# BerserkerMother/Video-Summarization

Hardware: AMD Instinct MI355X
Metric: frames/sec scored (whole node), synthetic [B,T=1024,D=1024] (higher is better)
Workload: dtype f32; 1 GPU; configs[2]: B=64 videos x T=1024 frames x D=1024 per GPU, scorer cfg M-A (heads 4, d_model 256, layers 4), logits + hidden state; global_batch=64, parallelism=videos sharded over 1 GPU(s), no all_gather of scores

## Files before the change

### video-summarization_amd/csrc/vs_kernels.hip

```cpp
#include "vs_train_device.h"
#include "vs_kernels.h"
#include "vs_launch.h"

namespace {

enum { EPI_BIAS = 0, EPI_RELU = 1, EPI_PE = 2, EPI_QKV = 3,
       EPI_GATE = 4,
       EPI_RELU_DROP = 5 };
struct EpiArgs {
    unsigned long long seed;
    unsigned site;
    float p;
    float scale;
};

__device__ __forceinline__ unsigned long long stamp() { return vs_stamp(); }

template <int EPI, int NWM = 2, int DIAG = 0, int NJ = 2, int PREC = 0, int C16 = 0, int KW = 32, int A16 = 0>
__global__ __launch_bounds__(128 * NWM, 2) void gemm_nt_128(
    const float *__restrict__ A, const float *__restrict__ W, const float *__restrict__ bias,
    float *__restrict__ C, int M, int N, int K, const float *__restrict__ pe, int T, int H, int dh,
    unsigned long long *__restrict__ diag = nullptr, EpiArgs ea = EpiArgs{0ull, 0u, 0.f, 0.f}) {
    static_assert(KW == 32 || (KW == 64 && (PREC == 1 || PREC == 3)), "64-wide k-tiles exist for the 16-bit operands only");
    static_assert(A16 == 0 || PREC == 1 || PREC == 3, "16-bit-stored A belongs to the 16-bit operand modes");
// ... 476 lines not shown
            const float v = (PREC == 2 ? acc[j][t] * (1.0f / F16X3_WS) : acc[j][t]) + bj[j] + res[(size_t)row * N + cbase + 32 * j];
            acc[j][t] = v;
            s += v;
        }
        part[t] = half_sum(s);
    }
    if (r == 0) {
#pragma unroll
        for (int t = 0; t < 16; ++t) red[wc * 64 + 32 * wr + acc_row(t, h)] = part[t];
    }
    __syncthreads();
    float mean[16];
#pragma unroll
    for (int t = 0; t < 16; ++t) {
        const int rl = 32 * wr + acc_row(t, h);
        mean[t] = (red[rl] + red[64 + rl]) * (1.0f / N);
    }
    __syncthreads();
#pragma unroll
    for (int t = 0; t < 16; ++t) {
        float s = 0.f;
#pragma unroll
        for (int j = 0; j < NB; ++j) { const float c = acc[j][t] - mean[t]; acc[j][t] = c; s += c * c; }
        part[t] = half_sum(s);
    }
    if (r == 0) {
#pragma unroll
        for (int t = 0; t < 16; ++t) red[wc * 64 + 32 * wr + acc_row(t, h)] = part[t];
    }
    __syncthreads();
#pragma unroll
    for (int t = 0; t < 16; ++t) {
        const int rl = 32 * wr + acc_row(t, h);
        const float rstd = 1.0f / sqrtf((red[rl] + red[64 + rl]) * (1.0f / N) + 1e-5f);
        const int row = m0 + rl;
#pragma unroll
        for (int j = 0; j < NB; ++j) {
            const float y = acc[j][t] * rstd * gj[j] + bej[j];
            acc[j][t] = y;
            if (row < M) out[(size_t)row * N + cbase + 32 * j] = y;
        }
    }
    if (score_w != nullptr) {
        for (int c = 0; c < num_classes; ++c) {
            __syncthreads();
            float wj[NB];
#pragma unroll
            for (int j = 0; j < NB; ++j) wj[j] = score_w[(size_t)c * N + cbase + 32 * j];
#pragma unroll
            for (int t = 0; t < 16; ++t) {
                float s = 0.f;
#pragma unroll
                for (int j = 0; j < NB; ++j) s += acc[j][t] * wj[j];
                part[t] = half_sum(s);
            }
            if (r == 0) {
#pragma unroll
                for (int t = 0; t < 16; ++t) red[wc * 64 + 32 * wr + acc_row(t, h)] = part[t];
            }
            __syncthreads();
            if (tid < 64) {
                const int row = m0 + tid;
                if (row < M) {
                    float s = red[tid] + red[64 + tid] + score_b[c];
                    if (sigmoid) s = 1.0f / (1.0f + expf(-s));
                    scores[(size_t)row * num_classes + c] = s;
                }
            }
        }
    }
}

struct LnTail {
    const float *W2, *b2;
    float *C2;
    int T, H, dhs;
};
struct LnPhase2 {
    const float *W, *bias, *gamma, *beta;
    float *out;
    LnTail tl;
};

template <int NT, int PREC, int A16, int DIAG, int TAIL>
__device__ __forceinline__ void ln_rows_tiles(
    const float *__restrict__ A, const float *__restrict__ W, const float *__restrict__ bias,
    const float *__restrict__ res, const float *__restrict__ gamma, const float *__restrict__ beta,
    float *__restrict__ out, int M, int K,
    const float *__restrict__ score_w, const float *__restrict__ score_b, int num_classes,
    int sigmoid, float *__restrict__ scores, unsigned long long *__restrict__ diag, const LnTail tl, const LnPhase2 p2) {
    static_assert(TAIL == 0 || (NT == 8 && PREC == 0 && DIAG == 0), "the register-fed tail exists for exact fp32 at d_model 256");
    constexpr int BM = 128, N = 32 * NT, BK = 16, LD = BK + 4;
    constexpr int WL = (N * BK / 4 + 255) / 256;
    constexpr bool TWO = TAIL >= 3;
    constexpr int NPH = TWO ? 2 : 1;
    constexpr int TN2 = TAIL == 2 ? 3 * N : 4 * N;
    constexpr int SMALL2 = TAIL == 3 ? 3 * N + 3 * N : TAIL == 4 ? 3 * N : 0;
    __shared__ __attribute__((aligned(16))) float smem[2 * (BM + N) * LD + 4 * N + (TAIL != 0 ? TN2 : 0) + SMALL2];
    float *gam_s = smem + 2 * (BM + N) * LD, *bet_s = gam_s + N, *sw_s = bet_s + N, *bias_s = sw_s + N;
    float *bias2_s = bias_s + N;
    float *small2_s = bias2_s + TN2;

    int tid = threadIdx.x, lane = tid & 63, wave = tid >> 6;
    int r = lane & 31, h = lane >> 5;
    const int ntiles = (M + BM - 1) / BM;
    const int nk = K / BK;

    constexpr float SC = PREC == 2 ? F16X3_WS : 1.0f;
    for (int i = tid; i < N; i += 256) { gam_s[i] = gamma[i]; bet_s[i] = beta[i]; bias_s[i] = bias[i] * SC; }
    if constexpr (TAIL != 0)
        for (int i = tid; i < TN2; i += 256) bias2_s[i] = tl.b2[i];
    if constexpr (TWO) {
        for (int i = tid; i < N; i += 256) { small2_s[i] = p2.gamma[i]; small2_s[N + i] = p2.beta[i]; small2_s[2 * N + i] = p2.bias[i]; }
        if constexpr (TAIL == 3)
            for (int i = tid; i < 3 * N; i += 256) small2_s[3 * N + i] = p2.tl.b2[i];
    }

    int lrow = tid >> 2, lc4 = (tid & 3) * 4;
    f32x4 pa[2], pw[WL];
    u32x2 pa16[2];
    const float *aptr[2], *wptr[WL];
    const unsigned short *aptr16[2];
#pragma unroll
    for (int i = 0; i < WL; ++i) {
        int wrow = lrow + 64 * i; wrow = wrow < N ? wrow : N - 1;
        wptr[i] = W + (size_t)wrow * K + lc4;
    }
    static_assert(PREC != 0 || N % 64 == 0, "the exact-fp32 staging map covers W without a guard");
    __amdgpu_buffer_rsrc_t ars = __builtin_amdgcn_make_buffer_rsrc(const_cast<float *>(A), 0, 0, 0x00020000);
    __amdgpu_buffer_rsrc_t wrs = __builtin_amdgcn_make_buffer_rsrc(const_cast<float *>(W), 0, N * K * 4, 0x00020000);
    int aoff[2], woff[WL];
#pragma unroll
    for (int i = 0; i < WL; ++i) woff[i] = ((lrow + 64 * i) * K + lc4) * 4;
    auto gload = [&](int i, int kb) __attribute__((always_inline)) {
        if (i < 2) pa[i] = __builtin_bit_cast(f32x4, __builtin_amdgcn_raw_buffer_load_b128(ars, aoff[i], kb, 0));
        else pw[i - 2] = __builtin_bit_cast(f32x4, __builtin_amdgcn_raw_buffer_load_b128(wrs, woff[i - 2], kb, 0));
    };
    constexpr int LDB = 12;
    auto stage = [&](int buf) __attribute__((always_inline)) {
        float *As = smem + buf * (BM + N) * LD, *Ws = As + BM * LD;
        if constexpr (PREC == 2) {
#pragma unroll
            for (int i = 0; i < 2; ++i) {
                u32x2 hi, lo;
                split_f16x4((const float *)&pa[i], hi, lo);
                *(u32x2 *)&As[(lrow + 64 * i) * LD + lc4 / 2] = hi;
                *(u32x2 *)&As[(lrow + 64 * i) * LD + 8 + lc4 / 2] = lo;
            }
#pragma unroll
            for (int i = 0; i < WL; ++i)
                if (lrow + 64 * i < N) {
                    u32x2 hi, lo;
                    const f32x4 ws = pw[i] * F16X3_WS;
                    split_f16x4((const float *)&ws, hi, lo);
                    *(u32x2 *)&Ws[(lrow + 64 * i) * LD + lc4 / 2] = hi;
                    *(u32x2 *)&Ws[(lrow + 64 * i) * LD + 8 + lc4 / 2] = lo;
                }
        } else if constexpr (PREC == 1) {
#pragma unroll
            for (int i = 0; i < 2; ++i) {
                u32x2 u;
                if constexpr (A16 != 0) u = pa16[i];
                else { u[0] = pack_bf16(pa[i][0], pa[i][1]); u[1] = pack_bf16(pa[i][2], pa[i][3]); }
                *(u32x2 *)&As[(lrow + 64 * i) * LDB + lc4 / 2] = u;
            }
#pragma unroll
            for (int i = 0; i < WL; ++i)
                if (lrow + 64 * i < N) {
                    u32x2 u; u[0] = pack_bf16(pw[i][0], pw[i][1]); u[1] = pack_bf16(pw[i][2], pw[i][3]);
                    *(u32x2 *)&Ws[(lrow + 64 * i) * LDB + lc4 / 2] = u;
                }
        } else {
#pragma unroll
            for (int i = 0; i < 2; ++i) *(f32x4 *)&As[(lrow + 64 * i) * LD + lc4] = pa[i];
#pragma unroll
            for (int i = 0; i < WL; ++i) *(f32x4 *)&Ws[(lrow + 64 * i) * LD + lc4] = pw[i];
        }
    };

    f32x16 acc[NT];

    constexpr int TCH = 128, TWB = 4 * 32 * 36, TBUF = TCH * 36;
    static_assert(TAIL == 0 || TWB + 2 * TBUF <= 2 * (BM + N) * LD, "corners and weight tiles fit the staging area");
    int r2 = tid >> 3, c2 = (tid & 7) * 4;
    __amdgpu_buffer_rsrc_t wrs2 = __builtin_amdgcn_make_buffer_rsrc(const_cast<float *>(tl.W2), 0, TN2 * N * 4, 0x00020000);
    const float *tbias_s = bias2_s;
    int woff2 = (r2 * N + c2) * 4;
    f32x4 pw2[4];
    f32x16 U[4];
    auto tail_soff = [&](int c, int kt) __attribute__((always_inline)) { return (TCH * c * N + 32 * kt) * 4; };
    auto tail_load = [&](int i, int soff) __attribute__((always_inline)) {
        pw2[i] = __builtin_bit_cast(f32x4, __builtin_amdgcn_raw_buffer_load_b128(wrs2, woff2, soff + 32 * i * N * 4, 0));
    };
    auto tail_stage = [&](int buf) __attribute__((always_inline)) {
#pragma unroll
        for (int i = 0; i < 4; ++i) *(f32x4 *)&smem[TWB + buf * TBUF + (r2 + 32 * i) * 36 + c2] = pw2[i];
    };
    auto bias_mfma = [&](int c) __attribute__((always_inline)) {
        const f32x16 zero = {0.f, 0.f, 0.f, 0.f, 0.f, 0.f, 0.f, 0.f, 0.f, 0.f, 0.f, 0.f, 0.f, 0.f, 0.f, 0.f};
#pragma unroll
        for (int jj = 0; jj < 4; ++jj) {
            const float bv = tbias_s[TCH * c + 32 * jj + r];
            U[jj] = MFMA32(h == 0 ? bv : 0.f, 1.0f, zero);
        }
    };
    auto tail_step = [&](auto ktc, int nsoff) __attribute__((always_inline)) {
        constexpr int kt = decltype(ktc)::value;
        const float *wp = smem + TWB + (kt & 1) * TBUF + r * 36 + 4 * h;
        float *wd = smem + TWB + ((kt + 1) & 1) * TBUF + r2 * 36 + c2;
        f32x4 fw[3];
        fw[0] = *(const f32x4 *)wp;
        fw[1] = *(const f32x4 *)(wp + 32 * 36);
        __builtin_amdgcn_sched_barrier(0);
#pragma unroll
        for (int t = 0; t < 16; ++t) {
            const int g = t / 4, jj = t % 4;
            if (t + 2 < 16) fw[(t + 2) % 3] = *(const f32x4 *)(wp + 32 * ((t + 2) % 4) * 36 + 8 * ((t + 2) / 4));
            if (t < 4) tail_load(t, nsoff);
            if (t >= 12) *(f32x4 *)(wd + 32 * (t - 12) * 36) = pw2[t - 12];
#pragma unroll
            for (int s2 = 0; s2 < 4; ++s2) U[jj] = MFMA32(fw[t % 3][s2], acc[kt][4 * g + s2], U[jj]);
            __builtin_amdgcn_sched_group_barrier(0x008, 1, 0);
            if (t + 2 < 16) __builtin_amdgcn_sched_group_barrier(0x100, 1, 0);
            if (t < 4) __builtin_amdgcn_sched_group_barrier(0x020, 1, 0);
            __builtin_amdgcn_sched_group_barrier(0x008, 3, 0);
            if (t >= 12) __builtin_amdgcn_sched_group_barrier(0x200, 1, 0);
            __builtin_amdgcn_sched_barrier(0);
        }
        __syncthreads();
    };

    unsigned long long dsum[3] = {0, 0, 0}, tbegin = 0, tq = 0, ktiles = 0;
    if constexpr (DIAG != 0) tbegin = stamp();
    for (int tile = blockIdx.x; tile < ntiles; tile += gridDim.x) {
        if constexpr (DIAG != 0) tq = stamp();
        const int m0 = tile * BM;
      static_for<NPH>([&](auto phc) __attribute__((always_inline)) {
        constexpr int PH = decltype(phc)::value;
        constexpr bool P1 = TWO && PH == 1;
        constexpr int PT = !TWO ? TAIL : PH == 0 ? 1 : TAIL == 3 ? 2 : 0;
        constexpr int PTN2 = PT == 2 ? 3 * N : 4 * N, TNC = PTN2 / TCH;
        const LnTail ptl = P1 ? p2.tl : tl;
        const float *pA = P1 ? tl.C2 : A;
        const int pK = P1 ? 4 * N : K, pnk = P1 ? 4 * N / BK : nk;
        const float *pgam_s = P1 ? small2_s : gam_s, *pbet_s = P1 ? small2_s + N : bet_s, *pbias_s = P1 ? small2_s + 2 * N : bias_s;
        float *pout = P1 ? p2.out : out;
        if constexpr (TWO) {
            asm volatile("" : "+v"(tid));
            lane = tid & 63; wave = tid >> 6; r = lane & 31; h = lane >> 5;
            lrow = tid >> 2; lc4 = (tid & 3) * 4; r2 = tid >> 3; c2 = (tid & 7) * 4; woff2 = (r2 * N + c2) * 4;
            wrs = __builtin_amdgcn_make_buffer_rsrc(const_cast<float *>(P1 ? p2.W : W), 0, N * pK * 4, 0x00020000);
#pragma unroll
            for (int i = 0; i < WL; ++i) woff[i] = ((lrow + 64 * i) * pK + lc4) * 4;
            if constexpr (PT != 0) {
                wrs2 = __builtin_amdgcn_make_buffer_rsrc(const_cast<float *>(ptl.W2), 0, PTN2 * N * 4, 0x00020000);
                tbias_s = P1 ? small2_s + 3 * N : bias2_s;
            }
        }
        int row = m0 + 32 * wave + r;
        const bool row_ok = row < M;
        row = row_ok ? row : M - 1;
#pragma unroll
        for (int i = 0; i < 2; ++i) {
            int ar = m0 + lrow + 64 * i; ar = ar < M ? ar : M - 1;
            if constexpr (A16 != 0) {
                aptr16[i] = (const unsigned short *)A + (size_t)ar * K + lc4;
                pa16[i] = *(const u32x2 *)aptr16[i];
            } else if constexpr (PREC == 0) {
                aoff[i] = ((ar - m0) * pK + lc4) * 4;
            } else {
                aptr[i] = A + (size_t)ar * K + lc4;
                pa[i] = *(const f32x4 *)aptr[i];
            }
        }
        if constexpr (PREC == 0) {
            ars = __builtin_amdgcn_make_buffer_rsrc(const_cast<float *>(pA + (size_t)m0 * pK), 0, (M - m0 < BM ? M - m0 : BM) * pK * 4, 0x00020000);
            if constexpr (P1) {
#pragma unroll
                for (int i = 2; i < 2 + WL; ++i) gload(i, 0);
                asm volatile("s_waitcnt vmcnt(0)" ::: "memory");
                __builtin_amdgcn_fence(__ATOMIC_RELEASE, "workgroup");
                __syncthreads();
                __builtin_amdgcn_fence(__ATOMIC_ACQUIRE, "workgroup");
#pragma unroll
                for (int i = 0; i < 2; ++i) gload(i, 0);
            } else {
#pragma unroll
                for (int i = 0; i < 2 + WL; ++i) gload(i, 0);
            }
        } else {
#pragma unroll
            for (int i = 0; i < WL; ++i) pw[i] = *(const f32x4 *)wptr[i];
        }
        if constexpr (!P1) {
            const float *rp = res + (size_t)row * N + 4 * h;
#pragma unroll
            for (int j = 0; j < NT; ++j)
#pragma unroll
                for (int q = 0; q < 4; ++q) {
                    f32x4 rv = *(const f32x4 *)(rp + 32 * j + 8 * q);
                    if constexpr (PREC == 2) rv *= SC;
#pragma unroll
                    for (int e = 0; e < 4; ++e) acc[j][4 * q + e] = rv[e];
                }
        }
        if constexpr (!P1) __syncthreads();
        stage(0);
        __syncthreads();
        if constexpr (DIAG != 0) { dsum[2] += stamp() - tq; ktiles += nk; }

        for (int kt = 0; kt < pnk; ++kt) {
            const int kn = kt + 1 < pnk ? kt + 1 : kt;
            const float *As = smem + (kt & 1) * (BM + N) * LD, *Ws = As + BM * LD;
            if constexpr (PREC == 2) {
                const float *arow = As + (32 * wave + r) * LD + 4 * h;
                const f16x8 ah = __builtin_bit_cast(f16x8, *(const u32x4 *)arow);
                const f16x8 al = __builtin_bit_cast(f16x8, *(const u32x4 *)(arow + 8));
#pragma unroll
                for (int i = 0; i < 2; ++i) pa[i] = *(const f32x4 *)(aptr[i] + kn * BK);
#pragma unroll
                for (int i = 0; i < WL; ++i) pw[i] = *(const f32x4 *)(wptr[i] + kn * BK);
#pragma unroll
                for (int j = 0; j < NT; ++j) {
                    const float *wrow = Ws + (32 * j + r) * LD + 4 * h;
                    const f16x8 wh = __builtin_bit_cast(f16x8, *(const u32x4 *)wrow);
                    const f16x8 wl = __builtin_bit_cast(f16x8, *(const u32x4 *)(wrow + 8));
                    acc[j] = MFMA_F16(wl, ah, acc[j]);
                    acc[j] = MFMA_F16(wh, al, acc[j]);
                    acc[j] = MFMA_F16(wh, ah, acc[j]);
                }
                stage((kt + 1) & 1);
                __syncthreads();
                continue;
            }
            if constexpr (PREC == 1) {
                const bf16x8 fa = __builtin_bit_cast(bf16x8, *(const u32x4 *)(As + (32 * wave + r) * LDB + 4 * h));
#pragma unroll
                for (int i = 0; i < 2; ++i) {
                    if constexpr (A16 != 0) pa16[i] = *(const u32x2 *)(aptr16[i] + kn * BK);
                    else pa[i] = *(const f32x4 *)(aptr[i] + kn * BK);
                }
#pragma unroll
                for (int i = 0; i < WL; ++i) pw[i] = *(const f32x4 *)(wptr[i] + kn * BK);
#pragma unroll
                for (int j = 0; j < NT; ++j) {
                    const bf16x8 fw = __builtin_bit_cast(bf16x8, *(const u32x4 *)(Ws + (32 * j + r) * LDB + 4 * h));
                    acc[j] = MFMA_BF16(fw, fa, acc[j]);
                }
                stage((kt + 1) & 1);
                __syncthreads();
                continue;
            }
            const float *ap = As + (32 * wave + r) * LD + 4 * h;
            const float *wp = Ws + r * LD + 4 * h;
            constexpr int NS = 2 * NT, NL = 2 + WL;
            constexpr int LPS = (NL + NT - 1) / NT;
            constexpr int WB = NS - (NL + LPS - 1) / LPS;
            static_assert(BK == 16 && (NL + LPS - 1) / LPS <= NT, "loads and LDS writes of a k-tile occupy distinct steps");
            f32x4 fa[2], fw[3];
            fa[0] = *(const f32x4 *)ap;
            fw[0] = *(const f32x4 *)wp;
            fw[1] = *(const f32x4 *)(wp + 32 * LD);
            fa[1] = *(const f32x4 *)(ap + 8);
            __builtin_amdgcn_sched_barrier(0);
#pragma unroll
            for (int t = 0; t < NS; ++t) {
                const int g = t / NT, j = t % NT;
                if (t + 2 < NS) fw[(t + 2) % 3] = *(const f32x4 *)(wp + 32 * ((t + 2) % NT) * LD + 8 * ((t + 2) / NT));
                int nld = 0, nwr = 0;
#pragma unroll
                for (int q = 0; q < LPS; ++q) {
                    const int il = t * LPS + q, iw = (t - WB) * LPS + q;
                    if (il < NL) { gload(il, kn * (BK * 4)); ++nld; }
                    if (t >= WB && iw < NL) {
                        float *Ad = smem + ((kt + 1) & 1) * (BM + N) * LD, *Wd = Ad + BM * LD;
                        if (iw < 2) *(f32x4 *)&Ad[(lrow + 64 * iw) * LD + lc4] = pa[iw];
                        else *(f32x4 *)&Wd[(lrow + 64 * (iw - 2)) * LD + lc4] = pw[iw - 2];
                        ++nwr;
                    }
                }
#pragma unroll
                for (int s2 = 0; s2 < 4; ++s2) acc[j] = MFMA32(fw[t % 3][s2], fa[g][s2], acc[j]);
                __builtin_amdgcn_sched_group_barrier(0x008, 1, 0);
                if (t + 2 < NS) __builtin_amdgcn_sched_group_barrier(0x100, 1, 0);
#pragma unroll
                for (int q = 0; q < LPS; ++q)
                    if (q < nld) __builtin_amdgcn_sched_group_barrier(0x020, 1, 0);
                __builtin_amdgcn_sched_group_barrier(0x008, 3, 0);
#pragma unroll
                for (int q = 0; q < LPS; ++q)
                    if (q < nwr) __builtin_amdgcn_sched_group_barrier(0x200, 1, 0);
                __builtin_amdgcn_sched_barrier(0);
            }
            if constexpr (DIAG != 0) {
                const unsigned long long tb = stamp();
                __syncthreads();
                dsum[0] += stamp() - tb;
            } else
                __syncthreads();
        }
        if constexpr (DIAG != 0) tq = stamp();
        if constexpr (PT != 0) {
#pragma unroll
            for (int i = 0; i < 4; ++i) tail_load(i, tail_soff(0, 0));
        }

        float sum = 0.f;
#pragma unroll
        for (int j = 0; j < NT; ++j) {
            float pj = 0.f;
#pragma unroll
            for (int q = 0; q < 4; ++q) {
                const f32x4 bv = *(const f32x4 *)&pbias_s[32 * j + 8 * q + 4 * h];
#pragma unroll
                for (int e = 0; e < 4; ++e) { acc[j][4 * q + e] += bv[e]; pj += acc[j][4 * q + e]; }
            }
            sum += pj;
        }
        sum = pair_sum(sum);
        const float mean = sum * (1.0f / N);
        float sq = 0.f;
#pragma unroll
        for (int j = 0; j < NT; ++j) {
            float pj = 0.f;
#pragma unroll
            for (int t = 0; t < 16; ++t) { const float c = acc[j][t] - mean; acc[j][t] = c; pj += c * c; }
            sq += pj;
        }
        sq = pair_sum(sq);
        const float rstd = 1.0f / sqrtf(sq * (1.0f / N) + 1e-5f * (SC * SC));
        float *tp = smem + wave * (32 * 36);
        const int trow = lane >> 3, tc4 = (lane & 7) * 4;
#pragma unroll
        for (int j = 0; j < NT; ++j) {
#pragma unroll
            for (int q = 0; q < 4; ++q) {
                const f32x4 gv = *(const f32x4 *)&pgam_s[32 * j + 8 * q + 4 * h];
                const f32x4 bv = *(const f32x4 *)&pbet_s[32 * j + 8 * q + 4 * h];
                f32x4 y;
#pragma unroll
                for (int e = 0; e < 4; ++e) { y[e] = acc[j][4 * q + e] * rstd * gv[e] + bv[e]; acc[j][4 * q + e] = y[e]; }
                if constexpr (!TWO || P1) *(f32x4 *)&tp[r * 36 + 8 * q + 4 * h] = y;
            }
            if constexpr (TWO && !P1) __builtin_amdgcn_sched_barrier(0);
            if constexpr (!TWO || P1) {
#pragma unroll
                for (int pq = 0; pq < 4; ++pq) {
                    const f32x4 v = *(const f32x4 *)&tp[(trow + 8 * pq) * 36 + tc4];
                    const int orow = m0 + 32 * wave + trow + 8 * pq;
                    if (orow < M) *(f32x4 *)(pout + (size_t)orow * N + 32 * j + tc4) = v;
                }
            }
        }
        if constexpr (!TWO || (P1 && TAIL == 4))
        if (score_w != nullptr) {
            for (int c = 0; c < num_classes; ++c) {
                __syncthreads();
                for (int i = tid; i < N; i += 256) sw_s[i] = score_w[(size_t)c * N + i];
                __syncthreads();
                float dot = 0.f;
#pragma unroll
                for (int j = 0; j < NT; ++j) {
                    float pj = 0.f;
#pragma unroll
                    for (int q = 0; q < 4; ++q) {
                        const f32x4 wv = *(const f32x4 *)&sw_s[32 * j + 8 * q + 4 * h];
#pragma unroll
                        for (int e = 0; e < 4; ++e) pj += acc[j][4 * q + e] * wv[e];
                    }
                    dot += pj;
                }
                dot = pair_sum(dot);
                if (h == 0 && row_ok) {
                    float sc = dot + score_b[c];
                    if (sigmoid) sc = 1.0f / (1.0f + expf(-sc));
                    scores[(size_t)row * num_classes + c] = sc;
                }
            }
        }
        if constexpr (DIAG != 0) dsum[1] += stamp() - tq;
        if constexpr (PT != 0) {
            tail_stage(0);
            int rowoff[4];
            __amdgpu_buffer_rsrc_t crs;
            if constexpr (PT == 1) {
                crs = __builtin_amdgcn_make_buffer_rsrc(ptl.C2 + (size_t)m0 * PTN2, 0, (M - m0 < BM ? M - m0 : BM) * PTN2 * 4, 0x00020000);
#pragma unroll
                for (int p = 0; p < 4; ++p) rowoff[p] = ((32 * wave + trow + 8 * p) * PTN2 + tc4) * 4;
            } else {
                crs = __builtin_amdgcn_make_buffer_rsrc(ptl.C2, 0, 0, 0x00020000);
#pragma unroll
                for (int p = 0; p < 4; ++p) {
                    const int orow = m0 + 32 * wave + trow + 8 * p;
                    const int bb = orow / ptl.T, tt = orow - bb * ptl.T;
                    rowoff[p] = orow < M ? (((bb * ptl.H * ptl.T + tt) << ptl.dhs) + tc4) * 4 : (int)0x80000000;
                }
            }
            bias_mfma(0);
            __syncthreads();
            for (int c = 0; c < TNC; ++c) {
                const int cn = c + 1 < TNC ? c + 1 : c;
                static_for<8>([&](auto ktc) __attribute__((always_inline)) {
                    constexpr int kt = decltype(ktc)::value;
                    tail_step(ktc, kt < 7 ? tail_soff(c, kt + 1) : tail_soff(cn, 0));
                });
                if constexpr (PT == 2) {
                    const int which = c >> 1;
                    crs = __builtin_amdgcn_make_buffer_rsrc(ptl.C2 + (size_t)which * M * N, 0, M * N * 4, 0x00020000);
                }
#pragma unroll
                for (int jj = 0; jj < 4; ++jj) {
                    __builtin_amdgcn_sched_barrier(0);
#pragma unroll
                    for (int q = 0; q < 4; ++q) {
                        f32x4 v;
#pragma unroll
                        for (int e = 0; e < 4; ++e) v[e] = PT == 1 ? relu1(U[jj][4 * q + e]) : U[jj][4 * q + e];
                        *(f32x4 *)&tp[r * 36 + 8 * q + 4 * h] = v;
                    }
                    int soff;
                    if constexpr (PT == 1) soff = (TCH * c + 32 * jj) * 4;
                    else {
                        const int cc = (TCH * c + 32 * jj) & (N - 1), head = cc >> ptl.dhs, e0 = cc - (head << ptl.dhs);
                        soff = (((head * ptl.T) << ptl.dhs) + e0) * 4;
                    }
#pragma unroll
                    for (int p = 0; p < 4; ++p) {
                        const f32x4 v = *(const f32x4 *)&tp[(trow + 8 * p) * 36 + tc4];
                        __builtin_amdgcn_raw_buffer_store_b128(__builtin_bit_cast(u32x4, v), crs, rowoff[p], soff, 0);
                    }
                }
                __builtin_amdgcn_sched_barrier(0);
                bias_mfma(cn);
            }
        }
      });
    }
    if constexpr (DIAG != 0) {
        if (diag != nullptr && lane == 0) {
            unsigned long long *o = diag + ((size_t)blockIdx.x * 4 + wave) * 8;
            o[0] = dsum[0]; o[1] = dsum[1]; o[2] = dsum[2]; o[3] = 0; o[4] = 0;
            o[5] = stamp() - tbegin; o[6] = ktiles; o[7] = tbegin;
        }
    }
}

template <int NT, int PREC = 0, int A16 = 0, int DIAG = 0>
__global__ __launch_bounds__(256, 2) void gemm_ln_rows(
    const float *__restrict__ A, const float *__restrict__ W, const float *__restrict__ bias,
    const float *__restrict__ res, const float *__restrict__ gamma, const float *__restrict__ beta,
    float *__restrict__ out, int M, int K,
    const float *__restrict__ score_w, const float *__restrict__ score_b, int num_classes,
    int sigmoid, float *__restrict__ scores, unsigned long long *__restrict__ diag = nullptr) {
    ln_rows_tiles<NT, PREC, A16, DIAG, 0>(A, W, bias, res, gamma, beta, out, M, K, score_w, score_b, num_classes, sigmoid, scores, diag,
                                          LnTail{nullptr, nullptr, nullptr, 0, 0, 0}, LnPhase2{});
}

__global__ __launch_bounds__(256, 2) void layer_outproj_ln_fc1(
    const float *__restrict__ A, const float *__restrict__ W, const float *__restrict__ bias,
    const float *__restrict__ res, const float *__restrict__ gamma, const float *__restrict__ beta,
    float *__restrict__ out, int M, int K, const float *__restrict__ W1, const float *__restrict__ b1, float *__restrict__ hidden) {
    ln_rows_tiles<8, 0, 0, 0, 1>(A, W, bias, res, gamma, beta, out, M, K, nullptr, nullptr, 0, 0, nullptr, nullptr,
                                 LnTail{W1, b1, hidden, 0, 0, 0}, LnPhase2{});
}
__global__ __launch_bounds__(256, 2) void layer_fc2_ln_qkv(
    const float *__restrict__ A, const float *__restrict__ W, const float *__restrict__ bias,
    const float *__restrict__ res, const float *__restrict__ gamma, const float *__restrict__ beta,
    float *__restrict__ out, int M, int K, const float *__restrict__ Wqkv, const float *__restrict__ bqkv, float *__restrict__ qkv,
    int T, int H, int dhs) {
    ln_rows_tiles<8, 0, 0, 0, 2>(A, W, bias, res, gamma, beta, out, M, K, nullptr, nullptr, 0, 0, nullptr, nullptr,
                                 LnTail{Wqkv, bqkv, qkv, T, H, dhs}, LnPhase2{});
}
struct LayerTailArgs {
    const float *att, *Wo, *bo, *res, *g1, *be1;
    const float *W1, *b1;
    float *hidden;
    const float *W2, *b2, *g2, *be2;
    float *out;
    int M;
};
__global__ __launch_bounds__(256, 2) void gemm_ln_rows_tail_qkv(const LayerTailArgs a, const float *__restrict__ Wqkv,
                                                         const float *__restrict__ bqkv, float *__restrict__ qkv, int T, int H, int dhs) {
    ln_rows_tiles<8, 0, 0, 0, 3>(a.att, a.Wo, a.bo, a.res, a.g1, a.be1, nullptr, a.M, 256, nullptr, nullptr, 0, 0, nullptr, nullptr,
                                 LnTail{a.W1, a.b1, a.hidden, 0, 0, 0}, LnPhase2{a.W2, a.b2, a.g2, a.be2, a.out, LnTail{Wqkv, bqkv, qkv, T, H, dhs}});
}
__global__ __launch_bounds__(256, 2) void gemm_ln_rows_tail_score(const LayerTailArgs a, const float *__restrict__ score_w,
                                                           const float *__restrict__ score_b, int num_classes, int sigmoid,
                                                           float *__restrict__ scores) {
    ln_rows_tiles<8, 0, 0, 0, 4>(a.att, a.Wo, a.bo, a.res, a.g1, a.be1, nullptr, a.M, 256, score_w, score_b, num_classes, sigmoid, scores, nullptr,
                                 LnTail{a.W1, a.b1, a.hidden, 0, 0, 0}, LnPhase2{a.W2, a.b2, a.g2, a.be2, a.out, LnTail{nullptr, nullptr, nullptr, 0, 0, 0}});
}

__device__ __forceinline__ void skinny_mainloop(f32x16 &acc, const float *__restrict__ ap,
                                                const float *__restrict__ wp, int K) {
    f32x4 a[4][4], w[4][4];
    auto load = [&](int set, int off) __attribute__((always_inline)) {
#pragma unroll
        for (int g = 0; g < 4; ++g) {
            a[set][g] = *(const f32x4 *)(ap + off + 8 * g);
            w[set][g] = *(const f32x4 *)(wp + off + 8 * g);
        }
    };
    auto mma = [&](int set) __attribute__((always_inline)) {
#pragma unroll
        for (int g = 0; g < 4; ++g)
#pragma unroll
            for (int st = 0; st < 4; ++st) acc = MFMA32(w[set][g][st], a[set][g][st], acc);
    };
    const int nc = K / 32;
    load(0, 0); load(1, 32); load(2, 64);
    for (int c = 0; c < nc - 4; c += 4) {
        load(3, 96);  mma(0);
        load(0, 128); mma(1);
        load(1, 160); mma(2);
        load(2, 192); mma(3);
        ap += 128; wp += 128;
    }
    load(3, 96);
    mma(0); mma(1); mma(2); mma(3);
}

template <int EPI>
__global__ __launch_bounds__(256) void skinny_gemm(
    const float *__restrict__ A, const float *__restrict__ W, const float *__restrict__ bias,
    float *__restrict__ C, int M, int N, int K, const float *__restrict__ pe, int T, int H, int dh, EpiArgs ea) {
    const int lane = threadIdx.x & 63, wave = threadIdx.x >> 6, r = lane & 31, h = lane >> 5;
    const int m0 = blockIdx.x * 32, n0 = blockIdx.y * 128 + 32 * wave;
    if (n0 >= N) return;
    const int row = m0 + r;
    const int arow = row < M ? row : M - 1;
    const float *ap = A + (size_t)arow * K + 4 * h, *wp = W + (size_t)(n0 + r) * K + 4 * h;
    const f32x16 zero = {0.f, 0.f, 0.f, 0.f, 0.f, 0.f, 0.f, 0.f, 0.f, 0.f, 0.f, 0.f, 0.f, 0.f, 0.f, 0.f};
    f32x16 acc = MFMA32(h == 0 ? bias[n0 + r] : 0.f, 1.0f, zero);
    skinny_mainloop(acc, ap, wp, K);
    if (row >= M) return;
    int bb = 0, tt = 0;
    if (EPI == EPI_PE || EPI == EPI_QKV) { bb = row / T; tt = row - bb * T; }
    int which = 0, head = 0, e0 = 0;
    if (EPI == EPI_QKV) { const int d = H * dh; which = n0 / d; const int c = n0 - which * d; head = c / dh; e0 = c - head * dh; }
#pragma unroll
    for (int q = 0; q < 4; ++q) {
        const int co = 8 * q + 4 * h;
        f32x4 v;
#pragma unroll
        for (int e = 0; e < 4; ++e) v[e] = acc[4 * q + e];
        if (EPI == EPI_RELU || EPI == EPI_RELU_DROP) {
#pragma unroll
            for (int e = 0; e < 4; ++e) v[e] = relu1(v[e]);
        }
        if (EPI == EPI_PE) {
            const f32x4 pv = *(const f32x4 *)(pe + (size_t)tt * N + n0 + co);
#pragma unroll
            for (int e = 0; e < 4; ++e) v[e] += pv[e];
        }
        if (EPI == EPI_GATE) {
            const f32x4 gv = *(const f32x4 *)(pe + (size_t)row * N + n0 + co);
#pragma unroll
            for (int e = 0; e < 4; ++e) v[e] = gv[e] > 0.f ? v[e] * ea.scale : 0.f;
        }
        if (EPI == EPI_RELU_DROP) {
            const DropSite dsite = drop_site(ea.seed, ea.site, ea.p);
            const unsigned rk = drop_rowkey(dsite, (unsigned)row);
#pragma unroll
            for (int e = 0; e < 4; ++e) v[e] = drop_keep(dsite, rk, (unsigned)(n0 + co + e)) ? v[e] * dsite.scale : 0.f;
        }
        if (EPI == EPI_QKV)
            *(f32x4 *)(C + (size_t)which * M * (H * dh) + (((size_t)bb * H + head) * T + tt) * dh + e0 + co) = v;
        else
            *(f32x4 *)(C + (size_t)row * N + n0 + co) = v;
    }
}

template <int NW>
__global__ __launch_bounds__(64 * NW) void skinny_ln(
// ... 711 lines not shown
        if (blocks < 0) return (int)hipErrorInvalidDevice;
        hipLaunchKernelGGL((gemm_nt_128<EPI, 4, 0, 2, 0>), dim3(blocks), dim3(512), 0, st, A, W, bias, C, M, N, K, pe, T, H, dh, nullptr, ea);
    } else {
        const int blocks = persistent_blocks(((M + 127) / 128) * ((N + 127) / 128), 2);
        if (blocks < 0) return (int)hipErrorInvalidDevice;
        hipLaunchKernelGGL((gemm_nt_128<EPI, 2, 0, 2, 0>), dim3(blocks), dim3(256), 0, st, A, W, bias, C, M, N, K, pe, T, H, dh, nullptr, ea);
    }
    VSK_CHECK_LAUNCH();
    return 0;
}

int vsk_linear(const float *A, const float *W, const float *Wf, const float *bias, float *C, int M, int N, int K,
               int relu, const float *pe, int T, int bf16, hipStream_t st) {
    if (bf16 & VSK_F16) {
        bf16 &= ~VSK_F16;
        if (pe != nullptr) return launch_gemm<EPI_PE, 3>(A, W, Wf, bias, C, M, N, K, pe, T, 0, 0, bf16, st);
        if (relu) return launch_gemm<EPI_RELU, 3>(A, W, Wf, bias, C, M, N, K, nullptr, 1, 0, 0, bf16, st);
        return launch_gemm<EPI_BIAS, 3>(A, W, Wf, bias, C, M, N, K, nullptr, 1, 0, 0, bf16, st);
    }
    if (pe != nullptr) return launch_gemm<EPI_PE>(A, W, Wf, bias, C, M, N, K, pe, T, 0, 0, bf16, st);
    if (relu) return launch_gemm<EPI_RELU>(A, W, Wf, bias, C, M, N, K, nullptr, 1, 0, 0, bf16, st);
    return launch_gemm<EPI_BIAS>(A, W, Wf, bias, C, M, N, K, nullptr, 1, 0, 0, bf16, st);
}

int vsk_linear_gate(const float *A, const float *W, const float *Wf, const float *bias, const float *gate, float scale,
                    float *C, int M, int N, int K, hipStream_t st, int bf16) {
    if (bf16 & VSK_F16) return launch_gemm<EPI_GATE, 3>(A, W, Wf, bias, C, M, N, K, gate, 1, 0, 0, bf16 & ~VSK_F16, st, EpiArgs{0ull, 0u, 0.f, scale});
    return launch_gemm<EPI_GATE>(A, W, Wf, bias, C, M, N, K, gate, 1, 0, 0, bf16, st, EpiArgs{0ull, 0u, 0.f, scale});
}

int vsk_linear_relu_dropout(const float *A, const float *W, const float *Wf, const float *bias, float *C, int M, int N,
                            int K, unsigned long long seed, unsigned site, float p, hipStream_t st, int bf16) {
    if (bf16 & VSK_F16) return launch_gemm<EPI_RELU_DROP, 3>(A, W, Wf, bias, C, M, N, K, nullptr, 1, 0, 0, bf16 & ~VSK_F16, st, EpiArgs{seed, site, p, 0.f});
    return launch_gemm<EPI_RELU_DROP>(A, W, Wf, bias, C, M, N, K, nullptr, 1, 0, 0, bf16, st, EpiArgs{seed, site, p, 0.f});
}

int vsk_pack_fragments(const float *W, float *Wf, int N, int K, hipStream_t st) {
    if (N % 32 || K % 8) return -1;
    hipLaunchKernelGGL(pack_fragments, dim3(256), dim3(256), 0, st, W, Wf, N, K);
    VSK_CHECK_LAUNCH();
    return 0;
}

__global__ void pack_fragments_batch(VskMatJobs jobs) {
    const int job = blockIdx.y;
    const float *__restrict__ W = jobs.in[job];
    float *__restrict__ Wf = jobs.out[job];
    const int N = jobs.rows[job], K = jobs.cols[job];
    const size_t total = (size_t)N * K / 4;
    for (size_t idx = (size_t)blockIdx.x * blockDim.x + threadIdx.x; idx < total; idx += (size_t)gridDim.x * blockDim.x) {
        const int lane = (int)(idx & 63);
        const size_t gi = idx >> 6;
        const int g = (int)(gi % (K / 8)), nb = (int)(gi / (K / 8));
        const int row = 32 * nb + (lane & 31), col = 8 * g + 4 * (lane >> 5);
        *(f32x4 *)(Wf + idx * 4) = *(const f32x4 *)(W + (size_t)row * K + col);
    }
}

int vsk_pack_fragments_batch(const VskMatJobs &jobs, hipStream_t st) {
    if (jobs.n < 1 || jobs.n > VskMatJobs::MAX) return -1;
    for (int i = 0; i < jobs.n; ++i) if (jobs.rows[i] % 32 || jobs.cols[i] % 8) return -1;
    hipLaunchKernelGGL(pack_fragments_batch, dim3(64, jobs.n), dim3(256), 0, st, jobs);
    VSK_CHECK_LAUNCH();
    return 0;
}

int vsk_pack_fragments_f16x3(const float *W, float *Wh, int N, int K, hipStream_t st) {
    if (N % 32 || K % 16) return -1;
    hipLaunchKernelGGL(pack_fragments_f16x3, dim3(256), dim3(256), 0, st, W, (unsigned *)Wh, N, K);
    VSK_CHECK_LAUNCH();
    return 0;
}

#ifdef VS_WITH_DIAG
int vsk_diag_gemm(const float *A, const float *W, const float *bias, float *C, int M, int N, int K,
                  int grid, unsigned long long *diag, hipStream_t st) {
    const char *mode = getenv("VS_DIAG_MODE"), *nw = getenv("VS_DIAG_NWM");
    const int m = mode ? atoi(mode) : 1, nwm = nw ? atoi(nw) : 2;
    int blocks = nwm == 4 ? persistent_blocks(((M + 255) / 256) * ((N + 127) / 128), 1)
                          : persistent_blocks(((M + 127) / 128) * ((N + 127) / 128), 2);
    if (blocks < 0) return (int)hipErrorInvalidDevice;
    if (grid > 0) blocks = grid;
    const char *dprec = getenv("VS_DIAG_PREC"), *dkern = getenv("VS_DIAG_KERNEL"), *dnj = getenv("VS_DIAG_NJ");
    if (dkern && dkern[0] == 'l') {
        if (N != 256 || K < N) return -1;
        blocks = persistent_blocks((M + 127) / 128);
        if (blocks > (M + 127) / 128) blocks = (M + 127) / 128;
        if (grid > 0) blocks = grid;
        if (diag == nullptr)
            hipLaunchKernelGGL((gemm_ln_rows<8, 0>), dim3(blocks), dim3(256), 0, st, A, W, bias, A, bias, bias, C, M, K, nullptr, nullptr, 0, 0, nullptr);
        else
            hipLaunchKernelGGL((gemm_ln_rows<8, 0, 0, 1>), dim3(blocks), dim3(256), 0, st, A, W, bias, A, bias, bias, C, M, K, nullptr, nullptr, 0, 0, nullptr, diag);
        VSK_CHECK_LAUNCH();
        return 0;
    }
    if (!dprec && dnj && atoi(dnj) == 4) {
        if (N % 256) return -1;
        blocks = grid > 0 ? grid : persistent_blocks(((M + 255) / 256) * (N / 256), 1);
#define VSK_DG4(D_) hipLaunchKernelGGL((gemm_nt_128<EPI_RELU, 4, D_, 4>), dim3(blocks), dim3(512), 0, st, A, W, bias, C, M, N, K, nullptr, 1, 0, 0, diag)
        if (diag == nullptr) VSK_DG4(0); else if (m == 2) VSK_DG4(2); else VSK_DG4(3);
#undef VSK_DG4
        VSK_CHECK_LAUNCH();
        return 0;
    }
    if (dprec && atoi(dprec) == 1) {
        blocks = grid > 0 ? grid : persistent_blocks(((M + 255) / 256) * (N / 256), 1);
        if (m == 2)
            hipLaunchKernelGGL((gemm_nt_128<EPI_RELU, 4, 2, 4, 1, 0, 64>), dim3(blocks), dim3(512), 0, st, A, W, bias, C, M, N, K, nullptr, 1, 0, 0, diag);
        else
            hipLaunchKernelGGL((gemm_nt_128<EPI_RELU, 4, 3, 4, 1, 0, 64>), dim3(blocks), dim3(512), 0, st, A, W, bias, C, M, N, K, nullptr, 1, 0, 0, diag);
        VSK_CHECK_LAUNCH();
        return 0;
    }
    if (dprec) {
        blocks = grid > 0 ? grid : persistent_blocks(((M + 255) / 256) * (N / 256), 1);
        if (m == 2)
            hipLaunchKernelGGL((gemm_nt_128<EPI_RELU, 4, 2, 4, 2>), dim3(blocks), dim3(512), 0, st, A, W, bias, C, M, N, K, nullptr, 1, 0, 0, diag);
        else
            hipLaunchKernelGGL((gemm_nt_128<EPI_RELU, 4, 3, 4, 2>), dim3(blocks), dim3(512), 0, st, A, W, bias, C, M, N, K, nullptr, 1, 0, 0, diag);
        VSK_CHECK_LAUNCH();
        return 0;
    }
#define VSK_DG(NWM_, D_) hipLaunchKernelGGL((gemm_nt_128<EPI_RELU, NWM_, D_, 2>), dim3(blocks), dim3(128 * NWM_), 0, st, A, W, bias, C, M, N, K, nullptr, 1, 0, 0, diag)
    if (diag == nullptr) { if (nwm == 4) VSK_DG(4, 0); else VSK_DG(2, 0); }
    else if (m == 1) { if (nwm == 4) VSK_DG(4, 1); else VSK_DG(2, 1); }
    else if (m == 2) { if (nwm == 4) VSK_DG(4, 2); else VSK_DG(2, 2); }
    else { if (nwm == 4) VSK_DG(4, 3); else VSK_DG(2, 3); }
#undef VSK_DG
    VSK_CHECK_LAUNCH();
    return 0;
}
#endif

int vsk_qkv(const float *h, const float *Wqkv, const float *Wf, const float *bqkv, float *qkv, int B, int T, int d,
            int H, int bf16, hipStream_t st, float qscale) {
    if (bf16 & VSK_F16)
        return launch_gemm<EPI_QKV, 3>(h, Wqkv, Wf, bqkv, qkv, B * T, 3 * d, d, nullptr, T, H, d / H, bf16 & ~VSK_F16, st,
                                       EpiArgs{0ull, 0u, 0.f, qscale});
    return launch_gemm<EPI_QKV>(h, Wqkv, Wf, bqkv, qkv, B * T, 3 * d, d, nullptr, T, H, d / H, bf16, st,
                                EpiArgs{0ull, 0u, 0.f, qscale});
}

int vsk_linear_res_ln(const float *A, const float *W, const float *Wf, const float *bias, const float *res,
                      const float *gamma, const float *beta, float *out, int M, int N, int K,
                      const float *score_w, const float *score_b, int num_classes, int sigmoid,
                      float *scores, int bf16, hipStream_t st) {
    if (bf16 == 2 && Wf != nullptr && M <= skinny_max_rows() && N <= 256 && N % 32 == 0 && K % 128 == 0) {
        const int blocks = (M + 31) / 32;
        int rc = 0;
        if (!vsk_pick_int<2, 4, 6, 8>(N / 32, [&](auto NW) {
                if ((rc = vsk_raise_lds<skinny2_ln<NW(), 2>>(SKINNY2_LDS_MAX)) != 0) return;
                hipLaunchKernelGGL((skinny2_ln<NW(), 2>), dim3(blocks), dim3(64 * NW()), skinny2_lds(K), st, A, Wf, bias, res, gamma, beta,
                                   out, M, K, score_w, score_b, num_classes, sigmoid, scores);
            }))
            return -1;
        if (rc) return rc;
        VSK_CHECK_LAUNCH();
        return 0;
    }
    const bool a16 = bf16 == (1 | VSK_STORE16);
    if (a16) bf16 = 1;
    if (bf16 == 1 && (N > 256 || N % 32)) return -1;
    if (bf16 && N <= 256) {
        if (N % 32) return -1;
        int blocks = persistent_blocks((M + 127) / 128);
        if (blocks < 0) return (int)hipErrorInvalidDevice;
// ... 114 lines not shown
```

Baseline: 12.38 million frames/s.

## Overlap tail-GEMM output stores with MFMAs via carry/drain steps in fused LN tail

In the fused LN + FFN/QKV tail kernels, the epilogue of each output chunk (relu, LDS staging of the corner tile, global stores) is no longer done serially after the MFMA loop. It is interleaved into the last k-step of the current chunk (drain) and the first k-step of the next chunk (carry) using a compile-time schedule plan and sched_group_barriers. The aim is to hide the store and LDS-transpose latency behind matrix instructions. It also adds timing instrumentation and a diag launcher for the tail kernel, at the cost of more register pressure and considerably more complex scheduling.

```diff
diff --git a/video-summarization_amd/csrc/vs_kernels.hip b/video-summarization_amd/csrc/vs_kernels.hip
--- a/video-summarization_amd/csrc/vs_kernels.hip
+++ b/video-summarization_amd/csrc/vs_kernels.hip
@@ -582,14 +582,32 @@
     LnTail tl;
 };
 
-template <int NT, int PREC, int A16, int DIAG, int TAIL>
+struct DrainPlan {
+    int wr[3][4], rd[3][4], st[3][4];
+};
+constexpr DrainPlan drain_plan() {
+    DrainPlan P{};
+    for (int p = 0; p < 3; ++p)
+        for (int q = 0; q < 4; ++q) {
+            const int b = 16 * p + 15;
+            P.wr[p][q] = b + 2 + q;
+            P.rd[p][q] = q < 3 ? b + 6 + q : b + 10;
+            P.st[p][q] = q < 3 ? b + 10 + q : b + 14;
+        }
+    return P;
+}
+
+template <int NT, int PREC, int A16, int DIAG, int TAIL, int DRAIN = 0>
 __device__ __forceinline__ void ln_rows_tiles(
     const float *__restrict__ A, const float *__restrict__ W, const float *__restrict__ bias,
     const float *__restrict__ res, const float *__restrict__ gamma, const float *__restrict__ beta,
     float *__restrict__ out, int M, int K,
     const float *__restrict__ score_w, const float *__restrict__ score_b, int num_classes,
     int sigmoid, float *__restrict__ scores, unsigned long long *__restrict__ diag, const LnTail tl, const LnPhase2 p2) {
-    static_assert(TAIL == 0 || (NT == 8 && PREC == 0 && DIAG == 0), "the register-fed tail exists for exact fp32 at d_model 256");
+    static_assert(TAIL == 0 || (NT == 8 && PREC == 0), "the register-fed tail exists for exact fp32 at d_model 256");
+    static_assert((DIAG == 0 || TAIL == 0 || TAIL >= 3) && (DRAIN == 0 || TAIL >= 3), "stamps and the draining last step: two-phase tail only");
+    constexpr bool KD = DIAG != 0 && TAIL == 0;
+    constexpr bool TD = DIAG != 0 && TAIL != 0;
     constexpr int BM = 128, N = 32 * NT, BK = 16, LD = BK + 4;
     constexpr int WL = (N * BK / 4 + 255) / 256;
     constexpr bool TWO = TAIL >= 3;
@@ -704,7 +722,24 @@
             U[jj] = MFMA32(h == 0 ? bv : 0.f, 1.0f, zero);
         }
     };
-    auto tail_step = [&](auto ktc, int nsoff) __attribute__((always_inline)) {
+    unsigned long long tcur[3] = {0, 0, 0}, tstart = 0;
+    auto tail_barrier = [&]() __attribute__((always_inline)) {
+        if constexpr (TD) {
+            const unsigned long long tb = stamp();
+            __syncthreads();
+            const unsigned long long ta = stamp();
+            tcur[0] += tb - tstart; tcur[1] += ta - tb; tstart = ta;
+        } else
+            __syncthreads();
+    };
+    auto tail_first_mfma = [&](int counted) __attribute__((always_inline)) {
+        if constexpr (TD) {
+            const unsigned long long s0 = stamp();
+            tcur[2] += counted ? s0 - tstart : 0ull;
+            tstart = s0;
+        }
+    };
+    auto tail_step = [&](auto ktc, int nsoff, int counted = 0) __attribute__((always_inline)) {
         constexpr int kt = decltype(ktc)::value;
         const float *wp = smem + TWB + (kt & 1) * TBUF + r * 36 + 4 * h;
         float *wd = smem + TWB + ((kt + 1) & 1) * TBUF + r2 * 36 + c2;
@@ -712,6 +747,7 @@
         fw[0] = *(const f32x4 *)wp;
         fw[1] = *(const f32x4 *)(wp + 32 * 36);
         __builtin_amdgcn_sched_barrier(0);
+        if constexpr (kt == 0) tail_first_mfma(counted);
 #pragma unroll
         for (int t = 0; t < 16; ++t) {
             const int g = t / 4, jj = t % 4;
@@ -727,13 +763,99 @@
             if (t >= 12) __builtin_amdgcn_sched_group_barrier(0x200, 1, 0);
             __builtin_amdgcn_sched_barrier(0);
         }
-        __syncthreads();
-    };
-
-    unsigned long long dsum[3] = {0, 0, 0}, tbegin = 0, tq = 0, ktiles = 0;
+        tail_barrier();
+    };
+    float *ctp = smem;
+    int ctrow = 0, ctc4 = 0;
+    auto corner_write = [&](int jj, int q, bool relu) __attribute__((always_inline)) {
+        f32x4 v;
+#pragma unroll
+        for (int e = 0; e < 4; ++e) v[e] = relu ? relu1(U[jj][4 * q + e]) : U[jj][4 * q + e];
+        *(f32x4 *)&ctp[r * 36 + 8 * q + 4 * h] = v;
+    };
+    auto corner_read = [&](int p) __attribute__((always_inline)) { return *(const f32x4 *)&ctp[(ctrow + 8 * p) * 36 + ctc4]; };
+    auto tail_step_carry = [&](int nsoff, int counted, __amdgpu_buffer_rsrc_t drs, const int *rowoff, int dsoff) __attribute__((always_inline)) {
+        const float *wp = smem + TWB + r * 36 + 4 * h;
+        float *wd = smem + TWB + TBUF + r2 * 36 + c2;
+        f32x4 fw[3], rb[4];
+        fw[0] = *(const f32x4 *)wp;
+        fw[1] = *(const f32x4 *)(wp + 32 * 36);
+        __builtin_amdgcn_sched_barrier(0);
+        tail_first_mfma(counted);
+        static_for<64>([&](auto mc) __attribute__((always_inline)) {
+            constexpr int m = decltype(mc)::value, t = m / 4, s2 = m % 4, g = t / 4, jj = t % 4;
+            {
+                U[jj] = MFMA32(fw[t % 3][s2], acc[0][4 * g + s2], U[jj]);
+                __builtin_amdgcn_sched_group_barrier(0x008, 1, 0);
+                if constexpr (s2 == 0) {
+                    if constexpr (t + 2 < 16) {
+                        fw[(t + 2) % 3] = *(const f32x4 *)(wp + 32 * ((t + 2) % 4) * 36 + 8 * ((t + 2) / 4));
+                        __builtin_amdgcn_sched_group_barrier(0x100, 1, 0);
+                    }
+                    if constexpr (t < 4) { tail_load(t, nsoff); __builtin_amdgcn_sched_group_barrier(0x020, 1, 0); }
+                }
+                if constexpr (s2 == 2 && t >= 4 && t < 8) { rb[t - 4] = corner_read(t - 4); __builtin_amdgcn_sched_group_barrier(0x100, 1, 0); }
+                if constexpr (s2 == 2 && t >= 6 && t < 10) {
+                    __builtin_amdgcn_raw_buffer_store_b128(__builtin_bit_cast(u32x4, rb[t - 6]), drs, rowoff[t - 6], dsoff, 0);
+                    __builtin_amdgcn_sched_group_barrier(0x040, 1, 0);
+                }
+                if constexpr (s2 == 3 && t >= 12) { *(f32x4 *)(wd + 32 * (t - 12) * 36) = pw2[t - 12]; __builtin_amdgcn_sched_group_barrier(0x200, 1, 0); }
+                __builtin_amdgcn_sched_barrier(0);
+            }
+        });
+        tail_barrier();
+    };
+    auto tail_step_drain = [&](int nsoff, __amdgpu_buffer_rsrc_t crs, const int *rowoff, const int *soff, bool relu,
+                               const float *nbias, float *bv) __attribute__((always_inline)) {
+        constexpr DrainPlan P = drain_plan();
+        const float *wp = smem + TWB + TBUF + r * 36 + 4 * h;
+        float *wd = smem + TWB + r2 * 36 + c2;
+        f32x4 fw[3], rb[4];
+        fw[0] = *(const f32x4 *)wp;
+        fw[1] = *(const f32x4 *)(wp + 8);
+        __builtin_amdgcn_sched_barrier(0);
+        static_for<64>([&](auto mc) __attribute__((always_inline)) {
+            constexpr int m = decltype(mc)::value, t = m / 4, s2 = m % 4, jj = t / 4, g = t % 4;
+            U[jj] = MFMA32(fw[t % 3][s2], acc[NT - 1][4 * g + s2], U[jj]);
+            __builtin_amdgcn_sched_group_barrier(0x008, 1, 0);
+            if constexpr (s2 == 0) {
+                if constexpr (t + 2 < 16) {
+                    fw[(t + 2) % 3] = *(const f32x4 *)(wp + 32 * ((t + 2) / 4) * 36 + 8 * ((t + 2) % 4));
+                    __builtin_amdgcn_sched_group_barrier(0x100, 1, 0);
+                }
+                if constexpr (t < 4) { tail_load(t, nsoff); __builtin_amdgcn_sched_group_barrier(0x020, 1, 0); }
+            }
+            static_for<12>([&](auto pqc) __attribute__((always_inline)) {
+                constexpr int p = decltype(pqc)::value / 4, q = decltype(pqc)::value % 4;
+                if constexpr (P.wr[p][q] == m) { corner_write(p, q, relu); __builtin_amdgcn_sched_group_barrier(0x200, 1, 0); }
+            });
+            static_for<12>([&](auto pqc) __attribute__((always_inline)) {
+                constexpr int p = decltype(pqc)::value / 4, q = decltype(pqc)::value % 4;
+                if constexpr (P.st[p][q] == m) {
+                    __builtin_amdgcn_raw_buffer_store_b128(__builtin_bit_cast(u32x4, rb[q]), crs, rowoff[q], soff[p], 0);
+                    __builtin_amdgcn_sched_group_barrier(0x040, 1, 0);
+                }
+            });
+            static_for<12>([&](auto pqc) __attribute__((always_inline)) {
+                constexpr int p = decltype(pqc)::value / 4, q = decltype(pqc)::value % 4;
+                if constexpr (P.rd[p][q] == m) { rb[q] = corner_read(q); __builtin_amdgcn_sched_group_barrier(0x100, 1, 0); }
+            });
+            if constexpr (m == 60 || m == 62) {
+                constexpr int i = m - 60;
+                bv[i] = nbias[32 * i]; bv[i + 1] = nbias[32 * (i + 1)];
+                __builtin_amdgcn_sched_group_barrier(0x100, 2, 0);
+            }
+            if constexpr (s2 == 3 && t >= 12) { *(f32x4 *)(wd + 32 * (t - 12) * 36) = pw2[t - 12]; __builtin_amdgcn_sched_group_barrier(0x200, 1, 0); }
+            __builtin_amdgcn_sched_barrier(0);
+        });
+        tail_barrier();
+    };
+
+    unsigned long long dsum[3] = {0, 0, 0}, tsum[6] = {0, 0, 0, 0, 0, 0}, tbegin = 0, tq = 0, ktiles = 0;
     if constexpr (DIAG != 0) tbegin = stamp();
     for (int tile = blockIdx.x; tile < ntiles; tile += gridDim.x) {
-        if constexpr (DIAG != 0) tq = stamp();
+        if constexpr (KD) tq = stamp();
+        if constexpr (TD) ++ktiles;
         const int m0 = tile * BM;
       static_for<NPH>([&](auto phc) __attribute__((always_inline)) {
         constexpr int PH = decltype(phc)::value;
@@ -807,7 +929,7 @@
         if constexpr (!P1) __syncthreads();
         stage(0);
         __syncthreads();
-        if constexpr (DIAG != 0) { dsum[2] += stamp() - tq; ktiles += nk; }
+        if constexpr (KD) { dsum[2] += stamp() - tq; ktiles += nk; }
 
         for (int kt = 0; kt < pnk; ++kt) {
             const int kn = kt + 1 < pnk ? kt + 1 : kt;
@@ -892,14 +1014,14 @@
                     if (q < nwr) __builtin_amdgcn_sched_group_barrier(0x200, 1, 0);
                 __builtin_amdgcn_sched_barrier(0);
             }
-            if constexpr (DIAG != 0) {
+            if constexpr (KD) {
                 const unsigned long long tb = stamp();
                 __syncthreads();
                 dsum[0] += stamp() - tb;
             } else
                 __syncthreads();
         }
-        if constexpr (DIAG != 0) tq = stamp();
+        if constexpr (KD) tq = stamp();
         if constexpr (PT != 0) {
 #pragma unroll
             for (int i = 0; i < 4; ++i) tail_load(i, tail_soff(0, 0));
@@ -978,7 +1100,7 @@
                 }
             }
         }
-        if constexpr (DIAG != 0) dsum[1] += stamp() - tq;
+        if constexpr (KD) dsum[1] += stamp() - tq;
         if constexpr (PT != 0) {
             tail_stage(0);
             int rowoff[4];
@@ -998,11 +1120,51 @@
             }
             bias_mfma(0);
             __syncthreads();
+            if constexpr (TD) tstart = stamp();
+            auto block_soff = [&](int c, int jj) __attribute__((always_inline)) {
+                if constexpr (PT == 1) return (TCH * c + 32 * jj) * 4;
+                else {
+                    const int cc = (TCH * c + 32 * jj) & (N - 1), head = cc >> ptl.dhs, e0 = cc - (head << ptl.dhs);
+                    return (((head * ptl.T) << ptl.dhs) + e0) * 4;
+                }
+            };
+            if constexpr (DRAIN != 0) {
+                ctp = tp; ctrow = trow; ctc4 = tc4;
+                __amdgpu_buffer_rsrc_t drs = __builtin_amdgcn_make_buffer_rsrc(ptl.C2, 0, 0, 0x00020000);
+                int dsoff = 0;
+                for (int c = 0; c < TNC; ++c) {
+                    const int cn = c + 1 < TNC ? c + 1 : c;
+                    if constexpr (PT == 2)
+                        crs = __builtin_amdgcn_make_buffer_rsrc(ptl.C2 + (size_t)(c >> 1) * M * N, 0, M * N * 4, 0x00020000);
+                    int soff[4];
+#pragma unroll
+                    for (int jj = 0; jj < 4; ++jj) soff[jj] = block_soff(c, jj);
+                    float bv[4];
+                    static_for<8>([&](auto ktc) __attribute__((always_inline)) {
+                        constexpr int kt = decltype(ktc)::value;
+                        if constexpr (kt == 0) tail_step_carry(tail_soff(c, 1), c > 0, drs, rowoff, dsoff);
+                        else if constexpr (kt < 7) tail_step(ktc, tail_soff(c, kt + 1));
+                        else tail_step_drain(tail_soff(cn, 0), crs, rowoff, soff, PT == 1, tbias_s + TCH * cn + r, bv);
+                    });
+#pragma unroll
+                    for (int q = 0; q < 4; ++q) corner_write(3, q, PT == 1);
+                    __builtin_amdgcn_sched_barrier(0);
+                    const f32x16 zero = {0.f, 0.f, 0.f, 0.f, 0.f, 0.f, 0.f, 0.f, 0.f, 0.f, 0.f, 0.f, 0.f, 0.f, 0.f, 0.f};
+#pragma unroll
+                    for (int jj = 0; jj < 4; ++jj) U[jj] = MFMA32(h == 0 ? bv[jj] : 0.f, 1.0f, zero);
+                    drs = crs; dsoff = soff[3];
+                }
+                __builtin_amdgcn_sched_barrier(0);
+#pragma unroll
+                for (int p = 0; p < 4; ++p)
+                    __builtin_amdgcn_raw_buffer_store_b128(__builtin_bit_cast(u32x4, corner_read(p)), drs, rowoff[p], dsoff, 0);
+                __builtin_amdgcn_sched_barrier(0);
+            } else
             for (int c = 0; c < TNC; ++c) {
                 const int cn = c + 1 < TNC ? c + 1 : c;
                 static_for<8>([&](auto ktc) __attribute__((always_inline)) {
                     constexpr int kt = decltype(ktc)::value;
-                    tail_step(ktc, kt < 7 ? tail_soff(c, kt + 1) : tail_soff(cn, 0));
+                    tail_step(ktc, kt < 7 ? tail_soff(c, kt + 1) : tail_soff(cn, 0), c > 0);
                 });
                 if constexpr (PT == 2) {
                     const int which = c >> 1;
@@ -1018,12 +1180,7 @@
                         for (int e = 0; e < 4; ++e) v[e] = PT == 1 ? relu1(U[jj][4 * q + e]) : U[jj][4 * q + e];
                         *(f32x4 *)&tp[r * 36 + 8 * q + 4 * h] = v;
                     }
-                    int soff;
-                    if constexpr (PT == 1) soff = (TCH * c + 32 * jj) * 4;
-                    else {
-                        const int cc = (TCH * c + 32 * jj) & (N - 1), head = cc >> ptl.dhs, e0 = cc - (head << ptl.dhs);
-                        soff = (((head * ptl.T) << ptl.dhs) + e0) * 4;
-                    }
+                    const int soff = block_soff(c, jj);
 #pragma unroll
                     for (int p = 0; p < 4; ++p) {
                         const f32x4 v = *(const f32x4 *)&tp[(trow + 8 * p) * 36 + tc4];
@@ -1033,10 +1190,22 @@
                 __builtin_amdgcn_sched_barrier(0);
                 bias_mfma(cn);
             }
+            if constexpr (TD) {
+                tcur[2] += stamp() - tstart;
+#pragma unroll
+                for (int i = 0; i < 3; ++i) { tsum[3 * PH + i] += tcur[i]; tcur[i] = 0; }
+            }
         }
       });
     }
-    if constexpr (DIAG != 0) {
+    if constexpr (TD) {
+        if (diag != nullptr && lane == 0) {
+            unsigned long long *o = diag + ((size_t)blockIdx.x * 4 + wave) * 8;
+#pragma unroll
+            for (int i = 0; i < 6; ++i) o[i] = tsum[i];
+            o[6] = stamp() - tbegin; o[7] = ktiles;
+        }
+    } else if constexpr (DIAG != 0) {
         if (diag != nullptr && lane == 0) {
             unsigned long long *o = diag + ((size_t)blockIdx.x * 4 + wave) * 8;
             o[0] = dsum[0]; o[1] = dsum[1]; o[2] = dsum[2]; o[3] = 0; o[4] = 0;
@@ -1081,15 +1250,23 @@
 };
 __global__ __launch_bounds__(256, 2) void gemm_ln_rows_tail_qkv(const LayerTailArgs a, const float *__restrict__ Wqkv,
                                                          const float *__restrict__ bqkv, float *__restrict__ qkv, int T, int H, int dhs) {
-    ln_rows_tiles<8, 0, 0, 0, 3>(a.att, a.Wo, a.bo, a.res, a.g1, a.be1, nullptr, a.M, 256, nullptr, nullptr, 0, 0, nullptr, nullptr,
+    ln_rows_tiles<8, 0, 0, 0, 3, 1>(a.att, a.Wo, a.bo, a.res, a.g1, a.be1, nullptr, a.M, 256, nullptr, nullptr, 0, 0, nullptr, nullptr,
                                  LnTail{a.W1, a.b1, a.hidden, 0, 0, 0}, LnPhase2{a.W2, a.b2, a.g2, a.be2, a.out, LnTail{Wqkv, bqkv, qkv, T, H, dhs}});
 }
 __global__ __launch_bounds__(256, 2) void gemm_ln_rows_tail_score(const LayerTailArgs a, const float *__restrict__ score_w,
                                                            const float *__restrict__ score_b, int num_classes, int sigmoid,
                                                            float *__restrict__ scores) {
-    ln_rows_tiles<8, 0, 0, 0, 4>(a.att, a.Wo, a.bo, a.res, a.g1, a.be1, nullptr, a.M, 256, score_w, score_b, num_classes, sigmoid, scores, nullptr,
+    ln_rows_tiles<8, 0, 0, 0, 4, 1>(a.att, a.Wo, a.bo, a.res, a.g1, a.be1, nullptr, a.M, 256, score_w, score_b, num_classes, sigmoid, scores, nullptr,
                                  LnTail{a.W1, a.b1, a.hidden, 0, 0, 0}, LnPhase2{a.W2, a.b2, a.g2, a.be2, a.out, LnTail{nullptr, nullptr, nullptr, 0, 0, 0}});
 }
+#ifdef VS_WITH_DIAG
+template <int DRAIN, int DIAG>
+__global__ __launch_bounds__(256, 2) void diag_tail_qkv(const LayerTailArgs a, const float *__restrict__ Wqkv, const float *__restrict__ bqkv,
+                                                        float *__restrict__ qkv, int T, int H, int dhs, unsigned long long *__restrict__ diag) {
+    ln_rows_tiles<8, 0, 0, DIAG, 3, DRAIN>(a.att, a.Wo, a.bo, a.res, a.g1, a.be1, nullptr, a.M, 256, nullptr, nullptr, 0, 0, nullptr, diag,
+                                           LnTail{a.W1, a.b1, a.hidden, 0, 0, 0}, LnPhase2{a.W2, a.b2, a.g2, a.be2, a.out, LnTail{Wqkv, bqkv, qkv, T, H, dhs}});
+}
+#endif
 
 __device__ __forceinline__ void skinny_mainloop(f32x16 &acc, const float *__restrict__ ap,
                                                 const float *__restrict__ wp, int K) {
@@ -1967,6 +2144,24 @@
     if (blocks < 0) return (int)hipErrorInvalidDevice;
     if (grid > 0) blocks = grid;
     const char *dprec = getenv("VS_DIAG_PREC"), *dkern = getenv("VS_DIAG_KERNEL"), *dnj = getenv("VS_DIAG_NJ");
+    if (dkern && dkern[0] == 't') {
+        if (K != 256 || N < 2304 || M % 1024) return -1;
+        const char *dd = getenv("VS_DIAG_DRAIN");
+        const int drain = dd ? atoi(dd) : 1;
+        blocks = persistent_blocks((M + 127) / 128);
+        if (blocks < 0) return (int)hipErrorInvalidDevice;
+        if (blocks > (M + 127) / 128) blocks = (M + 127) / 128;
+        if (grid > 0) blocks = grid;
+        const float *W1 = W + 256 * 256, *W2 = W1 + 1024 * 256;
+        float *rows = C + (size_t)M * 1024, *qkv = rows + (size_t)M * 256;
+        const LayerTailArgs a{A, W, bias, A, bias, bias, W1, bias, C, W2, bias, bias, bias, rows, M};
+#define VSK_DT(DR_, D_) hipLaunchKernelGGL((diag_tail_qkv<DR_, D_>), dim3(blocks), dim3(256), 0, st, a, W1, bias, qkv, 1024, 4, 6, diag)
+        if (diag == nullptr) { if (drain) VSK_DT(1, 0); else VSK_DT(0, 0); }
+        else { if (drain) VSK_DT(1, 1); else VSK_DT(0, 1); }
+#undef VSK_DT
+        VSK_CHECK_LAUNCH();
+        return 0;
+    }
     if (dkern && dkern[0] == 'l') {
         if (N != 256 || K < N) return -1;
         blocks = persistent_blocks((M + 127) / 128);
```

Result: no change. 12.40 million frames/s (median of 6 runs) (+0.2%).
